# Furyton/Recommender-Baseline-Model

Hardware: AMD Instinct MI355X
Metric: training sequences/sec, SASRec L=200 d=128 at 1/2/4/8 MI355X; HR@10 parity (higher is better)
Workload: dtype bf16; 1 GPU; SASRec ML-1M shape (|items|=3416, seq_len=200, d=128, 2 blocks, 1 head, dropout 0.2); model=SASRec, global_batch=128, per_gpu_batch=128, seq_len=200, hidden=128, blocks=2, heads=1, num_items=3416, parallelism=dp1, hip_graph=True, bench_config=cfg2, sampler=host, steps_per_graph=10, full=False

## Files before the change

### include/recsys_hip.h

```cpp
#ifndef RECSYS_HIP_H
#define RECSYS_HIP_H
#include <stdint.h>
#ifdef __cplusplus
extern "C" {
#endif

#define RS_ERR_ARG 1001
#define RS_ERR_UNSUPPORTED 1002

typedef struct rs_epilogue {
  const float* bias;
  float alpha;
  int act;
  const void* aux;
  void* aux_out;
  int64_t ldaux;
  float drop_p;
  uint64_t drop_seed;
  const uint64_t* seed_base;
  int64_t drop_ld;
  const void* resid;
  int64_t ldres;
  const int64_t* rowmask_ids;
  int accumulate;
// ... 205 lines not shown
                        float* part, void* stream);
int rs_sas_block_boundary_fused(int64_t M, int64_t d);
int rs_sas_block_out_in(int64_t M, int64_t d, const void* o, const void* Q, const void* Wo, const float* bo, void* x1,
                        const float* ln_w, const float* ln_b, float eps, void* z, float* mean, float* rstd,
                        const void* W1, const float* b1, void* h1, const void* W2, const float* b2, void* xn,
                        const int64_t* ids, float drop_p, uint64_t salt1, uint64_t salt2, const uint64_t* seed_base,
                        const float* ln1_w, const float* ln1_b, float eps1, void* Qn, float* mean1, float* rstd1,
                        const void* Wq, const float* bq, void* q, const void* Wkv, const float* bkv, void* kv,
                        void* stream);
int rs_sas_block_in_out_bwd(int64_t M, int64_t d, const void* dq, const void* dkv, const void* dx1, const void* x,
                            const float* mean1, const float* rstd1, const float* ln1_w, const void* WinT, void* dx,
                            float* part1, const int64_t* ids, const void* h1, const void* x1, const float* mean2,
                            const float* rstd2, const float* ln2_w, const void* W2T, const void* W1T, const void* WoT,
                            void* dy2, void* da1, void* dx1o, void* dout, float* part2, float drop_p, uint64_t salt1,
                            uint64_t salt2, const uint64_t* seed_base, const void* o, float* delta, void* stream);
int rs_transpose_bf16(int64_t nmat, const int64_t* desc, int64_t max_tiles, const void* src, void* dst,
                      void* stream);

typedef struct {
  const void* dY; int64_t lddy;
  const void* X;  int64_t ldx;
  int64_t N, K;
  float* dW;
  float* db;
} rs_wgrad_problem;
typedef struct {
  const float* src; int64_t stride; int64_t splits; int64_t n; float* out;
} rs_reduce_segment;
int64_t rs_wgrad_grouped_slab_numel(int nprob, const rs_wgrad_problem* probs, int64_t M, int64_t rows_per_split);
int rs_wgrad_grouped_tile(int nprob, const rs_wgrad_problem* probs);
// ... 83 lines not shown
```

### recommender-baseline-model_amd/_lib.py

```python
import ctypes as C
import os

import torch

PKG = os.path.dirname(os.path.abspath(__file__))
LIB_PATH = os.path.join(PKG, "librecsys_hip.so" if not os.environ.get("RS_LIB_VARIANT")
                        else f"librecsys_hip.{os.environ['RS_LIB_VARIANT']}.so")

F32, BF16 = 0, 1

i32, i64, u64, f32, f64, vp = C.c_int, C.c_int64, C.c_uint64, C.c_float, C.c_double, C.c_void_p


class Epilogue(C.Structure):
    _fields_ = [
        ("bias", vp), ("alpha", f32), ("act", i32),
        ("aux", vp), ("aux_out", vp), ("ldaux", i64),
        ("drop_p", f32), ("drop_seed", u64), ("seed_base", vp), ("drop_ld", i64),
        ("resid", vp), ("ldres", i64),
        ("rowmask_ids", vp), ("accumulate", i32),
        ("post_drop_p", f32), ("post_drop_seed", u64), ("rows_dev", vp),
    ]


# ... 72 lines not shown
                              u64, u64, vp, vp, vp, vp, vp, vp, vp, i64, vp, vp, vp, vp, vp, vp, vp, vp, vp, vp],
    "rs_sas_block_in_embed": [i64, i64, vp, i64, vp, vp, f32, f32, u64, vp, vp, vp, vp, vp, vp, f32, vp, vp, vp, vp,
                              vp, vp, vp, vp, vp, vp],
    "rs_sas_block_out": [i64, i64, vp, vp, vp, vp, vp, vp, vp, f32, vp, vp, vp, vp, vp, vp, vp, vp, vp, vp, f32,
                         u64, u64, vp, vp],
    "rs_sas_block_out_bwd": [i64, i64, vp, vp, vp, vp, vp, vp, vp, vp, vp, vp, vp, vp, vp, vp, vp, f32, u64, u64,
                             vp, vp],
    "rs_sas_block_out_bwd_delta": [i64, i64, vp, vp, vp, vp, vp, vp, vp, vp, vp, vp, vp, vp, vp, vp, vp, f32, u64,
                                   u64, vp, vp, vp, vp],
    "rs_sas_block_in_bwd": [i64, i64, vp, vp, vp, vp, vp, vp, vp, vp, vp, vp, vp],
    "rs_sas_block_boundary_fused": [i64, i64],
    "rs_sas_block_out_in": [i64, i64, vp, vp, vp, vp, vp, vp, vp, f32, vp, vp, vp, vp, vp, vp, vp, vp, vp, vp, f32,
                            u64, u64, vp, vp, vp, f32, vp, vp, vp, vp, vp, vp, vp, vp, vp, vp],
    "rs_sas_block_in_out_bwd": [i64, i64, vp, vp, vp, vp, vp, vp, vp, vp, vp, vp, vp, vp, vp, vp, vp, vp, vp, vp, vp,
                                vp, vp, vp, vp, vp, f32, u64, u64, vp, vp, vp, vp],
    "rs_wgrad_grouped": [i32, C.POINTER(WgradProblem), i64, i64, vp, i64, i32, C.POINTER(ReduceSegment), vp],
    "rs_reduce_segments": [i32, C.POINTER(ReduceSegment), i32, vp],
    "rs_wgrad_grouped_slab_numel": [i32, C.POINTER(WgradProblem), i64, i64],
    "rs_wgrad_grouped_tile": [i32, C.POINTER(WgradProblem)],
    "rs_wgrad_grouped_tile_max": [i32, C.POINTER(WgradProblem), i32],
    "rs_wgrad_grouped_max": [i32, C.POINTER(WgradProblem), i64, i64, vp, i64, i32, C.POINTER(ReduceSegment), i32, vp],
    "rs_item_index_ws_bytes": [i32, i64, i64, i64],
    "rs_item_index_build": [i32, vp, vp, vp, i64, i64, i64, vp, i64, vp],
    "rs_item_index_layout": [i32, i64, i64, i64, C.POINTER(i64)],
    "rs_sas_head_fwd": [i64, i64, vp, vp, vp, f32, vp, vp, vp, vp, vp, vp, vp, vp, vp, vp],
    "rs_sas_head_finish": [i64, vp, vp, vp, vp],
    "rs_sas_head_bwd": [i64, i64, vp, vp, vp, vp, vp, vp, vp, vp, vp, vp, vp, vp, vp, vp, vp, vp, vp, vp, vp],
    "rs_item_grad": [vp, i32, i64, i64, i64, vp, f32, f32, u64, vp, vp, vp, vp, vp, vp],
    "rs_item_grad_marked": [vp, i32, i64, i64, i64, vp, f32, f32, u64, vp, vp, vp, vp, vp, vp, vp, vp],
    "rs_item_grad_f32": [vp, i32, i64, i64, i64, vp, f32, f32, u64, vp, vp, vp, vp, vp, vp],
# ... 65 lines not shown
```

### recommender-baseline-model_amd/csrc/rowchain.hip

```cpp
#include "common.h"
#include "../../include/recsys_hip.h"

namespace rc {

#ifdef RC_PROF
__device__ unsigned long long g_rc_prof[4096 * 8 * 16];
#define RCPROF(slot)                                                                                 \
  do {                                                                                               \
    if ((threadIdx.x & 63) == 0) g_rc_prof[(blockIdx.x * 8 + (threadIdx.x >> 6)) * 16 + (slot)] = wall_clock64(); \
  } while (0)
#else
#define RCPROF(slot) \
  do {               \
  } while (0)
#endif

#ifndef RC_HEAD_PREFETCH
#define RC_HEAD_PREFETCH 1
#endif

#ifndef RC_NOSTORE
#define RC_NOSTORE 0
#endif

// ... 114 lines not shown
  for (int j = 0; j < Lay<D>::J; ++j)
#pragma unroll
    for (int e = 0; e < 4; ++e) {
      const float u = x.v[j][e] - mu;
      q += u * u;
    }
  rs = 1.0f / sqrtf(row_sum(q) / (float)D + eps);
#pragma unroll
  for (int j = 0; j < Lay<D>::J; ++j) {
    const f32x4 w = vec4<D>(gw, j, g), b = vec4<D>(gb, j, g);
#pragma unroll
    for (int e = 0; e < 4; ++e) x.v[j][e] = (x.v[j][e] - mu) * rs * w[e] + b[e];
  }
}

__device__ __forceinline__ float row16_sum(float v) { return row16_sum_up(v); }

template <int D>
__device__ __forceinline__ void ln_bwd(Act<D>& dy, const Raw<D>& xr, bool valid, const float* gw, float mu, float a,
                                       float* red, int lane, int wave) {
  const int g = lane >> 4, cl = lane & 15;
  float* rw = red + wave * 2 * D;
  float sg = 0.f, sgu = 0.f;
#pragma unroll
  for (int j = 0; j < Lay<D>::J; ++j) {
    const f32x4 w = vec4<D>(gw, j, g);
#pragma unroll
    for (int e = 0; e < 4; ++e) {
      const float gy = valid ? dy.v[j][e] : 0.f;
      const float u = (float)xr.v[j >> 1][4 * (j & 1) + e] - mu;
      const float gq = gy * w[e];
      const float pg = row16_sum(gy * (u * a)), pb = row16_sum(gy);
      if (cl == 0) {
        rw[feat(j, g, e)] += pg;
        rw[D + feat(j, g, e)] += pb;
      }
      sg += gq;
      sgu += gq * u;
      dy.v[j][e] = gq;
    }
  }
  sg = row_sum(sg);
  sgu = row_sum(sgu);
  const float mg = sg / (float)D, coef = a * a * a * sgu / (float)D;
#pragma unroll
  for (int j = 0; j < Lay<D>::J; ++j) asm volatile("" : "+v"(dy.v[j]));
#pragma unroll
  for (int j = 0; j < Lay<D>::J; ++j)
#pragma unroll
    for (int e = 0; e < 4; ++e)
      dy.v[j][e] = a * (dy.v[j][e] - mg) - coef * ((float)xr.v[j >> 1][4 * (j & 1) + e] - mu);
}

__device__ __forceinline__ void ln_zero(float* red, int D, int lane, int wave) {
  for (int i = lane; i < 2 * D; i += 64) red[wave * 2 * D + i] = 0.f;
}
template <int D>
__device__ __forceinline__ void ln_partials(const float* red, float* part, int tid) {
  __syncthreads();
  if (tid < 2 * D) {
    const int which = tid / D, c = tid % D;
    float s = 0.f;
#pragma unroll
    for (int w = 0; w < NW; ++w) s += red[(w * 2 + which) * D + c];
    part[((int64_t)blockIdx.x * 2 + which) * D + c] = s;
  }
// ... 75 lines not shown
}

struct OutFwd {
  bf16 *x1, *z, *h1, *xn;
  float *mean, *rstd;
  const int64_t* ids;
  float drop_p, eps;
  uint32_t s1, s2;
};
__device__ __forceinline__ void drop4(float p, uint32_t s32, int64_t m, int D, int j, int g, float (&dm)[4]) {
  const uint64_t idx = (uint64_t)(m * D + feat(j, g, 0));
  drop_mul2(p, s32, idx, dm[0], dm[1]);
  drop_mul2(p, s32, idx + 2, dm[2], dm[3]);
}
template <int D>
__device__ __forceinline__ void fwd_out_a(const Raw<D>& orr, const Raw<D>& Qr, const Tile& T, const bf16* wo,
                                          const bf16* w1, const float* lv, const OutFwd& o, Raw<D>& zr, Raw<D>& hr,
                                          int lane) {
  const int g = lane >> 4;
  Act<D> acc;
  Raw<D> r;
  zero<D>(acc);
  mm<D>(wo, orr, acc, lane);
#pragma unroll
  for (int j = 0; j < Lay<D>::J; ++j) {
    const f32x4 bb = vec4<D>(lv, j, g);
#pragma unroll
    for (int e = 0; e < 4; ++e) acc.v[j][e] = acc.v[j][e] + bb[e] + (float)Qr.v[j >> 1][4 * (j & 1) + e];
  }
  round_act<D>(acc, r);
  if (!RC_NOSTORE) store_raw<D>(o.x1, D, T.m, T.ok, r, g);
  float mu, rs;
  ln_fwd<D>(acc, lv + D, lv + 2 * D, o.eps, g, mu, rs);
  round_act<D>(acc, zr);
  if (!RC_NOSTORE) store_raw<D>(o.z, D, T.m, T.ok, zr, g);
  if (T.ok && g == 0) {
    o.mean[T.m] = mu;
    o.rstd[T.m] = rs;
  }
  zero<D>(acc);
  mm<D>(w1, zr, acc, lane);
  const bool drop = o.drop_p > 0.f;
#pragma unroll
  for (int j = 0; j < Lay<D>::J; ++j) {
    float dm[4] = {1.f, 1.f, 1.f, 1.f};
    if (drop) drop4(o.drop_p, o.s1, T.m, D, j, g, dm);
    const f32x4 bb = vec4<D>(lv + 3 * D, j, g);
#pragma unroll
    for (int e = 0; e < 4; ++e) acc.v[j][e] = fmaxf(acc.v[j][e] + bb[e], 0.f) * dm[e];
  }
  round_act<D>(acc, hr);
  if (!RC_NOSTORE) store_raw<D>(o.h1, D, T.m, T.ok, hr, g);
}
template <int D>
__device__ __forceinline__ void fwd_out_b(const Raw<D>& hr, const Raw<D>& zr, const Tile& T, const bf16* w2,
                                          const float* lv, const OutFwd& o, Raw<D>& xr, int lane, bool keep) {
  const int g = lane >> 4;
  Act<D> acc;
  zero<D>(acc);
  mm<D>(w2, hr, acc, lane);
  const bool drop = o.drop_p > 0.f;
#pragma unroll
  for (int j = 0; j < Lay<D>::J; ++j) {
    float dm[4] = {1.f, 1.f, 1.f, 1.f};
    if (drop) drop4(o.drop_p, o.s2, T.m, D, j, g, dm);
    const f32x4 bb = vec4<D>(lv + 4 * D, j, g);
#pragma unroll
// ... 228 lines not shown
__device__ __forceinline__ float h_sigmoid(float z) { return 1.f / (1.f + __expf(-z)); }

template <int D>
__device__ __forceinline__ int64_t head_rows(const HeadArgs& h, const Tile& T, Raw<D>& er, Raw<D>& nr, int g) {
  const int64_t ip = h.pos[T.mc], in = h.neg[T.mc];
  load_raw<D>(er, h.E, D, ip, g);
  load_raw<D>(nr, h.E, D, in, g);
  return ip;
}
template <int D>
__device__ __forceinline__ void head_rows_at(const HeadArgs& h, int64_t ip, int64_t in, Raw<D>& er, Raw<D>& nr,
                                             int g) {
  load_raw<D>(er, h.E, D, ip, g);
  load_raw<D>(nr, h.E, D, in, g);
}
template <int D>
__device__ __forceinline__ void head_tile(const Raw<D>& xr, const Raw<D>& er, const Raw<D>& nr, int64_t ip,
                                          const Tile& T, const float* gl, const float* bl, const HeadArgs& h,
                                          float scale, float* red, float (&acc)[3], int lane, int wave) {
  const int g = lane >> 4;
  Act<D> y;
  to_act<D>(y, xr);
  float mu, rs;
  ln_fwd<D>(y, gl, bl, h.eps, g, mu, rs);
  Raw<D> fr;
  round_act<D>(y, fr);
  store_raw<D>(h.f, D, T.m, T.ok, fr, g);
  float dp = 0.f, dn = 0.f;
#pragma unroll
  for (int j = 0; j < Lay<D>::J; ++j)
#pragma unroll
    for (int e = 0; e < 4; ++e) {
      dp += y.v[j][e] * (float)er.v[j >> 1][4 * (j & 1) + e];
      dn += y.v[j][e] * (float)nr.v[j >> 1][4 * (j & 1) + e];
    }
  dp = row_sum(dp);
  dn = row_sum(dn);
  const bool valid = T.ok && ip != 0;
  const float gp = valid ? (h_sigmoid(dp) - 1.f) * scale : 0.f;
// ... 3 lines not shown
    h.nl[T.m] = dn;
    h.dpl[T.m] = gp;
    h.dnl[T.m] = gn;
    if (ip != 0) {
      acc[0] += h_softplus(-dp);
      acc[1] += h_softplus(dn);
      acc[2] += 1.f;
    }
  }
  Act<D> df;
#pragma unroll
  for (int j = 0; j < Lay<D>::J; ++j)
#pragma unroll
    for (int e = 0; e < 4; ++e)
      df.v[j][e] = gp * (float)er.v[j >> 1][4 * (j & 1) + e] + gn * (float)nr.v[j >> 1][4 * (j & 1) + e];
  ln_bwd<D>(df, xr, T.ok, gl, mu, rs, red, lane, wave);
  Raw<D> dr;
  round_act<D>(df, dr);
  store_raw<D>(h.dx, D, T.m, T.ok, dr, g);
}
__device__ __forceinline__ OutFwd out_fwd_of(const OutArgs& a) {
  const bool drop = a.drop_p > 0.f;
  return OutFwd{a.x1, a.z, a.h1, a.xn, a.mean, a.rstd, a.ids, a.drop_p, a.eps,
                drop ? seed32(eff_seed(a.salt1, a.seed_base)) : 0u, drop ? seed32(eff_seed(a.salt2, a.seed_base)) : 0u};
}

template <int D, bool HEAD>
__global__ __launch_bounds__(NT) void block_out_kernel(OutArgs a) {
  extern __shared__ __attribute__((aligned(16))) char smem[];
  typedef Smem<D, 3, 7, 1> L;
  constexpr int WB = Lay<D>::WBYTES;
  const float* lv = reinterpret_cast<const float*>(smem + L::W);
  float* red = reinterpret_cast<float*>(smem + L::V);
  constexpr bool head = HEAD;
// ... 327 lines not shown
  }
  asm volatile("" ::: "memory");
  if (has) {
    as_loaded<D>(dxr);
    bwd_out_a<D>(dxr, hr, T, wimg(w3), ob, dzr, dar, lane, T.ok && id != 0);
  }
  if constexpr (R::ON) __syncthreads();
  asm volatile("" ::: "memory");
  if (has)
    bwd_out_b<D>(dar, x1r, dzr, orr, T, mu2, rs2, wimg(R::ON ? w0 : w4), wimg(R::ON ? w1 : w5), lv + D, ob, red2,
                 lane, wave);
  ln_partials<D>(red, a.part, tid);
  ln_partials<D>(red2, b.part, tid);
}

static int g_ncu = 0;
static int64_t grid_for(int64_t M) {
  if (g_ncu == 0) {
    int dev = 0, n = 0;
    if (hipGetDevice(&dev) == hipSuccess && hipDeviceGetAttribute(&n, hipDeviceAttributeMultiprocessorCount, dev) ==
                                                 hipSuccess && n > 0)
      g_ncu = n;
    else
      g_ncu = 256;
  }
  const int64_t nt = (M + TR - 1) / TR;
  return nt < g_ncu ? nt : g_ncu;
}
template <int D> static size_t lds_fwd() { return Smem<D, 3, 5, 0>::BYTES; }
template <int D, bool HEAD> static size_t lds_out() {
// ... 19 lines not shown
  else if (d == 128) head ? launch_out_t<128, true>(a, s) : launch_out_t<128, false>(a, s);
  else return RS_ERR_UNSUPPORTED;
  return (int)hipGetLastError();
}

static bool boundary_fused(int64_t M, int64_t d) {
  return M > 0 && (d == 64 || d == 128) && (M + TR - 1) / TR <= grid_for(M) * NW;
}
template <int D>
static void launch_out_in_t(const OutArgs& a, const InArgs& b, hipStream_t s) {
  hipLaunchKernelGGL(block_out_in_kernel<D>, dim3((unsigned)grid_for(a.M)), dim3(NT), 0, s, a, b);
}
template <int D>
static void launch_in_out_bwd_t(const InBwdArgs& a, const OutBwdArgs& b, hipStream_t s) {
  hipLaunchKernelGGL(block_in_out_bwd_kernel<D>, dim3((unsigned)grid_for(a.M)), dim3(NT), 0, s, a, b);
}

__global__ __launch_bounds__(256) void transpose_bf16_kernel(const int64_t* __restrict__ desc, const __bf16* src,
                                                             __bf16* dst) {
  __shared__ __bf16 t[64][66];
  const int64_t* dsc = desc + 6 * blockIdx.y;
  const int64_t rows = dsc[0], cols = dsc[1];
  const int64_t tc = cdiv(cols, 64);
  const int64_t tr = blockIdx.x / tc, tcc = blockIdx.x % tc;
  if (tr * 64 >= rows) return;
  const __bf16* sp = src + dsc[2];
  __bf16* dp = dst + dsc[4];
  const int64_t lds = dsc[3], ldd = dsc[5];
  for (int e = threadIdx.x; e < 64 * 64; e += 256) {
    const int r = e / 64, c = e % 64;
// ... 189 lines not shown
    if (rc1) return rc1;
    return rs_sas_block_out_bwd_delta(M, d, dx, ids, h1, x1p, mean2, rstd2, ln2_w, W2T, W1T, WoT, dy2, da1, dx1p, dout,
                                      part2, drop_p, salt1, salt2, seed_base, o, delta, stream);
  }
  rc::InBwdArgs a = {M, (const __bf16*)dq, (const __bf16*)dkv, (const __bf16*)dx1, (const __bf16*)x, mean1, rstd1,
                     ln1_w, (const __bf16*)WinT, 3 * d, nullptr, part1};
  rc::OutBwdArgs b = {M, nullptr, ids, (const __bf16*)h1, (const __bf16*)x1p, mean2, rstd2, ln2_w,
                      (const __bf16*)W2T, (const __bf16*)W1T, (const __bf16*)WoT, (__bf16*)dy2, (__bf16*)da1,
                      (__bf16*)dx1p, (__bf16*)dout, part2, drop_p, salt1, salt2, seed_base, (const __bf16*)o, delta};
  hipStream_t s = (hipStream_t)stream;
  if (d == 64) rc::launch_in_out_bwd_t<64>(a, b, s);
  else rc::launch_in_out_bwd_t<128>(a, b, s);
  return (int)hipGetLastError();
}

int rs_transpose_bf16(int64_t nmat, const int64_t* desc, int64_t max_tiles, const void* src, void* dst,
                      void* stream) {
  if (nmat <= 0 || max_tiles <= 0) return RS_ERR_ARG;
  hipLaunchKernelGGL(rc::transpose_bf16_kernel, dim3((unsigned)max_tiles, (unsigned)nmat), dim3(256), 0,
                     (hipStream_t)stream, desc, (const __bf16*)src, (__bf16*)dst);
  return (int)hipGetLastError();
}

}
```

### recommender-baseline-model_amd/models/sas_model/sas.py

```python
import math
import os

import torch
import torch.nn as nn

from ... import ops
from ...engine_util import Workspace, as_ids, capture_event, compute_dtype, require_cuda, site_salt
from ...flat import FlatParams

LN_EPS = 1e-8
SAS_LOSSES = ("bce", "ce")


class PointWiseFeedForward(nn.Module):

    def __init__(self, hidden_units, dropout_rate):
        super().__init__()
        self.conv1 = nn.Conv1d(hidden_units, hidden_units, kernel_size=1)
        self.conv2 = nn.Conv1d(hidden_units, hidden_units, kernel_size=1)
        self.dropout_rate = dropout_rate


class SAS(nn.Module):
    def __init__(self, args):
# ... 133 lines not shown
        self.d = model.hidden
        self.L = model.num_blocks
        self.H = model.heads
        self.Dh = self.d // self.H
        self.p = float(model.dropout_rate)
        self.dt = model.cdtype
        self.dev = flat.device
        if self.dt == torch.bfloat16:
            flat.enable_bf16()
        self.ws = Workspace(self.dev)
        self.seed_base = torch.zeros(1, dtype=torch.int64, device=self.dev)
        self.external_seed = False
        self.adam_transposes = False
        self._wT = None
        self.boundary_fuse = os.environ.get("RS_SAS_BOUNDARY_FUSE", "1") != "0"
        salt0 = int(torch.randint(0, 2 ** 62, (1,)).item())
        self.salt = {"emb": site_salt(salt0, 0)}
        for i in range(self.L):
            self.salt[f"attn{i}"] = site_salt(salt0, 1 + 4 * i)
            self.salt[f"ffn1_{i}"] = site_salt(salt0, 2 + 4 * i)
            self.salt[f"ffn2_{i}"] = site_salt(salt0, 3 + 4 * i)

    def sync_compute_weights(self):
        f = self.flat
        if f.bf16 is not None:
            if not f.stale:
                ops.cast_bf16(f.data, f.bf16)
            else:
                a = 0
                for lo, hi in sorted(f.stale) + [(f.numel, f.numel)]:
# ... 148 lines not shown
            ops.sas_block_in(x, ln_w, ln_b, LN_EPS, Q, mu1, r1, Wq, bq, q, Wkv, bkv, kv)
        if after_first is not None:
            after_first()
        xs = [x]
        for i in range(L):
            b = lay[i]
            ops.attn_fwd(B, T, H, Dh, b["q"], b["kv"][:, :d], b["kv"][:, d:], b["o"], b["lse"], 1.0 / math.sqrt(Dh),
                         0, ids, p, self.salt[f"attn{i}"], sb)
            if i + 1 < L:
                ln_w, ln_b, Q, mu1, r1, Wq, bq, q, Wkv, bkv, kv = in_args(i + 1)
                if self.boundary_fuse:
                    ops.sas_block_out_in(out_args(i), ln_w, ln_b, LN_EPS, Q, mu1, r1, Wq, bq, q, Wkv, bkv, kv)
                else:
                    ops.sas_block_out(*out_args(i))
                    ops.sas_block_in(b["xn"], ln_w, ln_b, LN_EPS, Q, mu1, r1, Wq, bq, q, Wkv, bkv, kv)
            elif head is not None:
                ops.sas_block_out_head(out_args(i), *head)
            else:
                ops.sas_block_out(*out_args(i))
            xs.append(b["xn"])
        for i in range(L):
            b = lay[i]
            for k_ in ("Q", "mu1", "r1", "q", "kv", "o", "lse", "x1", "z", "mu2", "r2", "h1"):
                s[k_].append(b[k_])
            s["x"].append(xs[i])
        return xs[L]

    @property
    def fused_head(self):
        return ops.sas_block_fused_ok(self.d, self.dt)
# ... 5 lines not shown
        e = self._buf
        G = lambda n: self.flat.view(n, grad)
        slab = self.ws.get("slab", (ops.wgrad_slab_numel(M, 2 * d, d),), torch.float32)
        wln = self.ws.get("ln", (2 * 512 * d,), torch.float32)
        wat = self.ws.get("attn", (B * H * T,), torch.float32)

        fused = ops.sas_block_fused_ok(d, self.dt)
        if fused:
            ev, iws = s["side"] if "side" in s else self._side_prologue(ids, s["pos"], s["neg"])
        if fused:
            dx = e("dx", (M, d))
            lnh = self.ws.get("lnh", (2 * d * (-(-M // 64)),), torch.float32)
            E, gl = self.W("item_emb.weight"), self.Wf("last_layernorm.weight")
            stats = ()
            nb = -(-M // 64)
            if dpl is None and "head_in_block" in s:
                assert s["hdiv"] is divisor, "backward's divisor must be the one forward's head used"
                dx, dpl, dnl, lnh = s["hdx"], s["dpl"], s["dnl"], s["lnh"]
                nb = s["headp"].numel() // 3
                if loss_out is not None:
                    stats = (s["headp"], divisor, loss_out) + ((aux_out,) if aux_out is not None else ())
            elif dpl is None:
                dpl, dnl = e("dpl", (B, T), torch.float32), e("dnl", (B, T), torch.float32)
                ops.sas_head_bwd(s["headp"], divisor, loss_out, s["pl"], s["nl"], None, None, dpl, dnl, s["pos"],
                                 s["neg"], E, s["xL"], gl, s["muf"], s["rf"], dx, lnh)
            else:
                ops.sas_head_bwd(None, None, None, None, None, dpl, dnl, None, None, s["pos"], s["neg"], E, s["xL"],
                                 gl, s["muf"], s["rf"], dx, lnh)
            segs = ops.ln_partial_segments(lnh, M, d, G("last_layernorm.weight"), G("last_layernorm.bias"), nb=nb)
            if self._side_refreshed:
# ... 219 lines not shown
        if self._wT is None:
            self._wT = torch.empty(L * 6 * d * d, dtype=torch.bfloat16, device=self.dev)
            desc = []
            for i in range(L):
                base = i * 6 * d * d
                pre, fw = f"attention_layers.{i}.", f"forward_layers.{i}."
                for name, rows, off in ((pre + "in_proj_weight", 3 * d, 0), (pre + "out_proj.weight", d, 3 * d * d),
                                        (fw + "conv1.weight", d, 4 * d * d), (fw + "conv2.weight", d, 5 * d * d)):
                    desc.append([rows, d, self.flat.offsets[name], d, base + off, rows])
            self._wT_desc = torch.tensor(desc, dtype=torch.int64, device=self.dev)
            self._wT_desc_host = desc
            self._wT_tiles = max(-(-r // 64) * -(-c // 64) for r, c, *_ in desc)
        ops.transpose_bf16(self._wT_desc, self._wT_tiles, self.flat.bf16, self._wT)
        return self._wT

    def _backward_blocks_fused(self, s, dx, grad, extra_segs=(), tail=None, pos=None):
        B, T, p, ids, sb = s["B"], s["T"], s["p"], s["ids"], s["sb"]
        M, d, H, Dh, L = B * T, self.d, self.H, self.Dh, self.L
        e = self._buf
        G = lambda n: self.flat.view(n, grad)
        wT = self._wT.view(L, 6, d, d)
        nb = ops.sas_block_parts(M)
        lnp = self.ws.get("lnp", (L, 2, 2 * d * nb), torch.float32)
        wat = self.ws.get("attn", (B * H * T,), torch.float32)
        probs, segs = [], list(extra_segs)
        g = [dict(dy2=e("dy2", (M, d)), da1=e("da1", (M, d)), dx1=e("dx1", (M, d)), do=e("do", (M, d)),
                  dq=e("dq", (M, d)), dkv=e("dkv", (M, 2 * d))) for _ in range(L)]

        dl = [self.ws.get(f"attn_delta{i}", (B * H * T,), torch.float32) for i in range(L)] if H == 1 else None

        def out_bwd_args(i):
            return (ids, s["h1"][i], s["x1"][i], s["mu2"][i], s["r2"][i], self.Wf(f"forward_layernorms.{i}.weight"),
                    wT[i, 5], wT[i, 4], wT[i, 3], g[i]["dy2"], g[i]["da1"], g[i]["dx1"], g[i]["do"], lnp[i, 0], p,
                    self.salt[f"ffn1_{i}"], self.salt[f"ffn2_{i}"], sb, s["o"][i] if dl else None, dl[i] if dl else None)

        def in_bwd_args(i):
            return (g[i]["dq"], g[i]["dkv"], g[i]["dx1"], s["x"][i], s["mu1"][i], s["r1"][i],
                    self.Wf(f"attention_layernorms.{i}.weight"), wT[i, 0:3].reshape(d, 3 * d))

        ops.sas_block_out_bwd(dx, *out_bwd_args(L - 1))
        for i in reversed(range(L)):
            pre, fw = f"attention_layers.{i}.", f"forward_layers.{i}."
            dq, dkv, kv = g[i]["dq"], g[i]["dkv"], s["kv"][i]
            ops.attn_bwd(B, T, H, Dh, s["q"][i], kv[:, :d], kv[:, d:], s["o"][i], g[i]["do"], s["lse"][i], dq,
                         dkv[:, :d], dkv[:, d:], 1.0 / math.sqrt(Dh), 0, ids, p, self.salt[f"attn{i}"], sb,
                         dl[i] if dl else wat, delta_in=bool(dl))
            if i > 0 and self.boundary_fuse:
                dxi = None if ops.sas_block_boundary_fused(M, d) else e("dxi", (M, d))
                ops.sas_block_in_out_bwd(in_bwd_args(i), dxi, lnp[i, 1], out_bwd_args(i - 1))
            else:
                dxi = e("dxi", (M, d))
                ops.sas_block_in_bwd(*in_bwd_args(i), dxi, lnp[i, 1])
                if i > 0:
                    ops.sas_block_out_bwd(dxi, *out_bwd_args(i - 1))
            dx = dxi
# ... 52 lines not shown
```

### recommender-baseline-model_amd/ops.py

```python
import ctypes as C
import os

import torch

from . import _lib
from ._lib import BF16, F32, Epilogue, call, ptr, stream

ACT_NONE, ACT_RELU, ACT_GELU, ACT_RELU_BWD, ACT_GELU_BWD = (
    _lib.ACT_NONE, _lib.ACT_RELU, _lib.ACT_GELU, _lib.ACT_RELU_BWD, _lib.ACT_GELU_BWD)


STAMP_KINDS = {1: "attn_bwd", 2: "wgrad_grouped", 3: "vocab_ce_fwd"}


def kernel_stamps(buf, step, kinds=()):
    mask = sum(1 << k for k, n in STAMP_KINDS.items() if n in kinds)
    call("rs_kernel_stamps", ptr(buf), ptr(step), mask)


def read_kernel_stamps(buf, khz):
    import numpy as np
    h = buf.cpu().numpy().view(np.uint64)
    steps, marks, W = int(h[1]), int(h[2]), int(h[3])
    rec = h[4:4 + steps * marks * (1 + W)].reshape(steps, marks, 1 + W)
# ... 504 lines not shown
         ptr(seed_base), ptr(ln1_w), ptr(ln1_b), eps1, ptr(Qn), ptr(mean1), ptr(rstd1), ptr(Wq), ptr(bq), ptr(q),
         ptr(Wkv), ptr(bkv), ptr(kv), stream())


def sas_block_in_out_bwd(in_args, dx, part1, out_args):
    dq, dkv, dx1, x, mean1, rstd1, ln1_w, WinT = in_args
    (ids, h1, x1, mean2, rstd2, ln2_w, W2T, W1T, WoT, dy2, da1, dx1o, dout, part2, drop_p, salt1, salt2,
     seed_base, o, delta) = out_args
    M, d = dq.shape
    call("rs_sas_block_in_out_bwd", M, d, ptr(dq), ptr(dkv), ptr(dx1), ptr(x), ptr(mean1), ptr(rstd1), ptr(ln1_w),
         ptr(WinT), ptr(dx), ptr(part1), ptr(ids), ptr(h1), ptr(x1), ptr(mean2), ptr(rstd2), ptr(ln2_w), ptr(W2T),
         ptr(W1T), ptr(WoT), ptr(dy2), ptr(da1), ptr(dx1o), ptr(dout), ptr(part2), drop_p, salt1, salt2,
         ptr(seed_base), ptr(o), ptr(delta), stream())


def touched_rows_ws_numel(rows):
    return int(_lib.lib().rs_touched_rows_ws_numel(rows))


def touched_rows(ids, rows, flags, index, count, ws):
    call("rs_touched_rows", ptr(ids), ids.numel(), rows, ptr(flags), ptr(index), ptr(count), ptr(ws), stream())


def rows_pack(src, index, count, compact):
    rows, d = src.shape
    call("rs_rows_pack", ptr(src), rows, d, ptr(index), ptr(count), ptr(compact), compact.shape[0], stream())


def rows_unpack(dst, index, compact):
    rows, d = dst.shape
# ... 250 lines not shown
```

Measured before the change: 481,300 sequences/s.

## Fuse last block output, BCE head, and first backward step into one kernel

New measurement: 498,200 sequences/s, median of 6. +3.5%, better.

```diff
diff --git a/include/recsys_hip.h b/include/recsys_hip.h
--- a/include/recsys_hip.h
+++ b/include/recsys_hip.h
@@ -243,6 +243,15 @@
                             const float* rstd2, const float* ln2_w, const void* W2T, const void* W1T, const void* WoT,
                             void* dy2, void* da1, void* dx1o, void* dout, float* part2, float drop_p, uint64_t salt1,
                             uint64_t salt2, const uint64_t* seed_base, const void* o, float* delta, void* stream);
+int rs_sas_block_out_head_bwd(int64_t M, int64_t d, const void* o, const void* Q, const void* Wo, const float* bo,
+                              void* x1, const float* ln_w, const float* ln_b, float eps, void* z, float* mean,
+                              float* rstd, const void* W1, const float* b1, void* h1, const void* W2, const float* b2,
+                              void* xn, const int64_t* ids, float drop_p, uint64_t salt1, uint64_t salt2,
+                              const uint64_t* seed_base, const void* E, const int64_t* pos, const int64_t* neg,
+                              const float* lnl_w, const float* lnl_b, const int* count_parts, int64_t ncount,
+                              const float* divisor, void* f, float* pl, float* nl, float* dpl, float* dnl, void* dx,
+                              float* lnpart, float* part, const void* W2T, const void* W1T, const void* WoT, void* dy2,
+                              void* da1, void* dx1, void* dout, float* part2, float* delta, void* stream);
 int rs_transpose_bf16(int64_t nmat, const int64_t* desc, int64_t max_tiles, const void* src, void* dst,
                       void* stream);
 
diff --git a/recommender-baseline-model_amd/_lib.py b/recommender-baseline-model_amd/_lib.py
--- a/recommender-baseline-model_amd/_lib.py
+++ b/recommender-baseline-model_amd/_lib.py
@@ -110,6 +110,9 @@
                             u64, u64, vp, vp, vp, f32, vp, vp, vp, vp, vp, vp, vp, vp, vp, vp],
     "rs_sas_block_in_out_bwd": [i64, i64, vp, vp, vp, vp, vp, vp, vp, vp, vp, vp, vp, vp, vp, vp, vp, vp, vp, vp, vp,
                                 vp, vp, vp, vp, vp, f32, u64, u64, vp, vp, vp, vp],
+    "rs_sas_block_out_head_bwd": [i64, i64, vp, vp, vp, vp, vp, vp, vp, f32, vp, vp, vp, vp, vp, vp, vp, vp, vp, vp,
+                                  f32, u64, u64, vp, vp, vp, vp, vp, vp, vp, i64, vp, vp, vp, vp, vp, vp, vp, vp, vp,
+                                  vp, vp, vp, vp, vp, vp, vp, vp, vp, vp],
     "rs_wgrad_grouped": [i32, C.POINTER(WgradProblem), i64, i64, vp, i64, i32, C.POINTER(ReduceSegment), vp],
     "rs_reduce_segments": [i32, C.POINTER(ReduceSegment), i32, vp],
     "rs_wgrad_grouped_slab_numel": [i32, C.POINTER(WgradProblem), i64, i64],
diff --git a/recommender-baseline-model_amd/csrc/rowchain.hip b/recommender-baseline-model_amd/csrc/rowchain.hip
--- a/recommender-baseline-model_amd/csrc/rowchain.hip
+++ b/recommender-baseline-model_amd/csrc/rowchain.hip
@@ -152,9 +152,47 @@
   }
 }
 
+template <int D>
+__device__ __forceinline__ void ln_fwd_head(Act<D>& x, const float* gw, const float* gb, float eps, int g, float& mu,
+                                            float& rs) {
+  float s = 0.f;
+#pragma unroll
+  for (int j = 0; j < Lay<D>::J; ++j)
+#pragma unroll
+    for (int e = 0; e < 4; ++e) s += x.v[j][e];
+  mu = row_sum(s) / (float)D;
+  float q = 0.f, u0 = 0.f;
+#pragma unroll
+  for (int j = 0; j < Lay<D>::J; ++j)
+#pragma unroll
+    for (int e = 0; e < 4; ++e) {
+      const float u = x.v[j][e] - mu;
+      if (j == 0 && e == 0) {
+        u0 = u;
+      } else if (j == 0 && e == 1) {
+        float sq = u * u;
+        asm volatile("" : "+v"(sq));
+        q = __builtin_fmaf(u0, u0, sq);
+      } else if ((j & 1) == 0 && e < 2) {
+        q = __builtin_fmaf(u, u, q);
+      } else {
+        float sq = u * u;
+        asm volatile("" : "+v"(sq));
+        q += sq;
+      }
+    }
+  rs = 1.0f / sqrtf(row_sum(q) / (float)D + eps);
+#pragma unroll
+  for (int j = 0; j < Lay<D>::J; ++j) {
+    const f32x4 w = vec4<D>(gw, j, g), b = vec4<D>(gb, j, g);
+#pragma unroll
+    for (int e = 0; e < 4; ++e) x.v[j][e] = (x.v[j][e] - mu) * rs * w[e] + b[e];
+  }
+}
+
 __device__ __forceinline__ float row16_sum(float v) { return row16_sum_up(v); }
 
-template <int D>
+template <int D, bool HEAD_FORM = false>
 __device__ __forceinline__ void ln_bwd(Act<D>& dy, const Raw<D>& xr, bool valid, const float* gw, float mu, float a,
                                        float* red, int lane, int wave) {
   const int g = lane >> 4, cl = lane & 15;
@@ -173,8 +211,13 @@
         rw[feat(j, g, e)] += pg;
         rw[D + feat(j, g, e)] += pb;
       }
-      sg += gq;
-      sgu += gq * u;
+      if constexpr (HEAD_FORM) {
+        sg = __builtin_fmaf(gy, w[e], sg);
+        sgu = __builtin_fmaf(u, gq, sgu);
+      } else {
+        sg += gq;
+        sgu += gq * u;
+      }
       dy.v[j][e] = gq;
     }
   }
@@ -186,8 +229,21 @@
 #pragma unroll
   for (int j = 0; j < Lay<D>::J; ++j)
 #pragma unroll
-    for (int e = 0; e < 4; ++e)
-      dy.v[j][e] = a * (dy.v[j][e] - mg) - coef * ((float)xr.v[j >> 1][4 * (j & 1) + e] - mu);
+    for (int e = 0; e < 4; ++e) {
+      const float u = (float)xr.v[j >> 1][4 * (j & 1) + e] - mu;
+      if constexpr (HEAD_FORM) {
+        float p1 = a * (dy.v[j][e] - mg), p2 = coef * u;
+        if ((j & 1) == 0 && e < 2) {
+          asm volatile("" : "+v"(p1), "+v"(p2));
+          dy.v[j][e] = p1 - p2;
+        } else {
+          asm volatile("" : "+v"(p2));
+          dy.v[j][e] = __builtin_fmaf(a, dy.v[j][e] - mg, -p2);
+        }
+      } else {
+        dy.v[j][e] = a * (dy.v[j][e] - mg) - coef * u;
+      }
+    }
 }
 
 __device__ __forceinline__ void ln_zero(float* red, int D, int lane, int wave) {
@@ -293,12 +349,11 @@
   drop_mul2(p, s32, idx + 2, dm[2], dm[3]);
 }
 template <int D>
-__device__ __forceinline__ void fwd_out_a(const Raw<D>& orr, const Raw<D>& Qr, const Tile& T, const bf16* wo,
-                                          const bf16* w1, const float* lv, const OutFwd& o, Raw<D>& zr, Raw<D>& hr,
-                                          int lane) {
+__device__ __forceinline__ void fwd_out_a_x(const Raw<D>& orr, const Raw<D>& Qr, const Tile& T, const bf16* wo,
+                                            const bf16* w1, const float* lv, const OutFwd& o, Raw<D>& zr, Raw<D>& hr,
+                                            int lane, Raw<D>& r, float& mu, float& rs) {
   const int g = lane >> 4;
   Act<D> acc;
-  Raw<D> r;
   zero<D>(acc);
   mm<D>(wo, orr, acc, lane);
 #pragma unroll
@@ -309,7 +364,6 @@
   }
   round_act<D>(acc, r);
   if (!RC_NOSTORE) store_raw<D>(o.x1, D, T.m, T.ok, r, g);
-  float mu, rs;
   ln_fwd<D>(acc, lv + D, lv + 2 * D, o.eps, g, mu, rs);
   round_act<D>(acc, zr);
   if (!RC_NOSTORE) store_raw<D>(o.z, D, T.m, T.ok, zr, g);
@@ -330,6 +384,14 @@
   }
   round_act<D>(acc, hr);
   if (!RC_NOSTORE) store_raw<D>(o.h1, D, T.m, T.ok, hr, g);
+}
+template <int D>
+__device__ __forceinline__ void fwd_out_a(const Raw<D>& orr, const Raw<D>& Qr, const Tile& T, const bf16* wo,
+                                          const bf16* w1, const float* lv, const OutFwd& o, Raw<D>& zr, Raw<D>& hr,
+                                          int lane) {
+  Raw<D> r;
+  float mu, rs;
+  fwd_out_a_x<D>(orr, Qr, T, wo, w1, lv, o, zr, hr, lane, r, mu, rs);
 }
 template <int D>
 __device__ __forceinline__ void fwd_out_b(const Raw<D>& hr, const Raw<D>& zr, const Tile& T, const bf16* w2,
@@ -588,15 +650,17 @@
   load_raw<D>(er, h.E, D, ip, g);
   load_raw<D>(nr, h.E, D, in, g);
 }
-template <int D>
-__device__ __forceinline__ void head_tile(const Raw<D>& xr, const Raw<D>& er, const Raw<D>& nr, int64_t ip,
-                                          const Tile& T, const float* gl, const float* bl, const HeadArgs& h,
-                                          float scale, float* red, float (&acc)[3], int lane, int wave) {
+template <int D, bool STORE_DX>
+__device__ __forceinline__ void head_tile_x(const Raw<D>& xr, const Raw<D>& er, const Raw<D>& nr, int64_t ip,
+                                            const Tile& T, const float* gl, const float* bl, const HeadArgs& h,
+                                            float scale, float* red, float (&acc)[3], int lane, int wave,
+                                            Raw<D>& dxr) {
   const int g = lane >> 4;
   Act<D> y;
   to_act<D>(y, xr);
   float mu, rs;
-  ln_fwd<D>(y, gl, bl, h.eps, g, mu, rs);
+  if constexpr (STORE_DX) ln_fwd<D>(y, gl, bl, h.eps, g, mu, rs);
+  else ln_fwd_head<D>(y, gl, bl, h.eps, g, mu, rs);
   Raw<D> fr;
   round_act<D>(y, fr);
   store_raw<D>(h.f, D, T.m, T.ok, fr, g);
@@ -630,10 +694,18 @@
 #pragma unroll
     for (int e = 0; e < 4; ++e)
       df.v[j][e] = gp * (float)er.v[j >> 1][4 * (j & 1) + e] + gn * (float)nr.v[j >> 1][4 * (j & 1) + e];
-  ln_bwd<D>(df, xr, T.ok, gl, mu, rs, red, lane, wave);
+  ln_bwd<D, !STORE_DX>(df, xr, T.ok, gl, mu, rs, red, lane, wave);
   Raw<D> dr;
   round_act<D>(df, dr);
-  store_raw<D>(h.dx, D, T.m, T.ok, dr, g);
+  if (STORE_DX) store_raw<D>(h.dx, D, T.m, T.ok, dr, g);
+  dxr = dr;
+}
+template <int D>
+__device__ __forceinline__ void head_tile(const Raw<D>& xr, const Raw<D>& er, const Raw<D>& nr, int64_t ip,
+                                          const Tile& T, const float* gl, const float* bl, const HeadArgs& h,
+                                          float scale, float* red, float (&acc)[3], int lane, int wave) {
+  Raw<D> dr;
+  head_tile_x<D, true>(xr, er, nr, ip, T, gl, bl, h, scale, red, acc, lane, wave, dr);
 }
 __device__ __forceinline__ OutFwd out_fwd_of(const OutArgs& a) {
   const bool drop = a.drop_p > 0.f;
@@ -991,6 +1063,123 @@
   ln_partials<D>(red2, b.part, tid);
 }
 
+struct TurnArgs {
+  OutArgs a;
+  OutBwdArgs b;
+};
+typedef const __attribute__((address_space(4))) TurnArgs* TurnArgsPtr;
+__device__ __forceinline__ TurnArgsPtr turn_args_late() {
+  TurnArgsPtr kp = (TurnArgsPtr)__builtin_amdgcn_kernarg_segment_ptr();
+  asm volatile("" : "+s"(kp));
+  return kp;
+}
+template <int D>
+__global__ __launch_bounds__(NT) void block_out_head_bwd_kernel(TurnArgs k) {
+  const OutArgs& a = k.a;
+  typedef Roll<D> R;
+  RC_BOUNDARY_SLOTS(D);
+  __shared__ __attribute__((aligned(16))) float lv[7 * D];
+  __shared__ __attribute__((aligned(16))) float red[NW * 2 * D], red2[NW * 2 * D];
+  __shared__ float hred[4][NW];
+  const int tid = threadIdx.x, lane = tid & 63, wave = __builtin_amdgcn_readfirstlane(tid >> 6), g = lane >> 4,
+            cl = lane & 15;
+  RCPROF(0);
+  const TileRange tr = tiles_of_wave(n_tiles(a.M), wave);
+  const bool has = tr.first < tr.end;
+  const Tile T = tile_of(has ? tr.first : 0, a.M, cl);
+  const OutFwd of = out_fwd_of(a);
+  Raw<D> orr, Qr;
+  int64_t id = 0, ip = 0, in = 0;
+  if (has) {
+    load_raw<D>(orr, a.o, D, T.mc, g);
+    load_raw<D>(Qr, a.Q, D, T.mc, g);
+    id = a.ids[T.mc];
+    ip = a.h.pos[T.mc];
+    in = a.h.neg[T.mc];
+  }
+  stage_slot<D>(w0, a.Wo, D, wave, lane);
+  stage_slot<D>(w1, a.W1, D, wave, lane);
+  stage_slot<D>(w2, a.W2, D, wave, lane);
+  stage_slot<D>(w3, k.b.W2T, D, wave, lane);
+  if constexpr (!R::ON) {
+    stage_slot<D>(w4, k.b.W1T, D, wave, lane);
+    stage_slot<D>(w5, k.b.WoT, D, wave, lane);
+  }
+  {
+    const float* const V[7] = {a.bo, a.ln_w, a.ln_b, a.b1, a.b2, a.h.gl, a.h.bl};
+    stage_v<D, 7>(lv, V, tid);
+  }
+  ln_zero(red, D, lane, wave);
+  ln_zero(red2, D, lane, wave);
+  float hacc[3] = {0.f, 0.f, 0.f};
+  {
+    int c = 0;
+    for (int i = tid; i < a.h.ncnt; i += NT) c += a.h.cnt_parts[i];
+    c = (int)wave_sum((float)c);
+    if (lane == 0) hred[3][wave] = (float)c;
+  }
+  __syncthreads();
+  float hscale;
+  {
+    float c = 0.f;
+#pragma unroll
+    for (int w = 0; w < NW; ++w) c += hred[3][w];
+    hscale = 1.f / (a.h.divisor ? *a.h.divisor : c);
+  }
+  asm volatile("" : "+v"(id), "+v"(ip), "+v"(in));
+  RCPROF(1);
+  Raw<D> zr, hr, x1r, xr, er, nr, dr, dzr, dar;
+  float mu2 = 0.f, rs2 = 0.f;
+  if (has) {
+    fwd_out_a_x<D>(orr, Qr, T, wimg(w0), wimg(w1), lv, of, zr, hr, lane, x1r, mu2, rs2);
+    head_rows_at<D>(a.h, ip, in, er, nr, g);
+  }
+  RCPROF(2);
+  if constexpr (R::ON) {
+    __syncthreads();
+    const TurnArgsPtr kp = turn_args_late();
+    stage_slot<D>(w0, kp->b.W1T, D, wave, lane);
+    stage_slot<D>(w1, kp->b.WoT, D, wave, lane);
+  }
+  asm volatile("" ::: "memory");
+  const TurnArgsPtr kb = turn_args_late();
+  const OutBwd ob = {kb->b.dy2, kb->b.da1, kb->b.dx1, kb->b.dout, kb->b.delta, a.ids, a.drop_p, of.s1, of.s2};
+  if (has) {
+    const bool keep = T.ok && id != 0;
+    fwd_out_b<D>(hr, zr, T, wimg(w2), lv, of, xr, lane, keep);
+    RCPROF(4);
+    head_tile_x<D, false>(xr, er, nr, ip, T, lv + 5 * D, lv + 6 * D, a.h, hscale, red, hacc, lane, wave, dr);
+    RCPROF(6);
+    asm volatile("" ::: "memory");
+    as_loaded<D>(dr);
+    as_loaded<D>(hr);
+    bwd_out_a<D>(dr, hr, T, wimg(w3), ob, dzr, dar, lane, keep);
+  }
+  if constexpr (R::ON) __syncthreads();
+  asm volatile("" ::: "memory");
+  if (has) {
+    as_loaded<D>(x1r);
+    as_loaded<D>(orr);
+    asm volatile("" : "+v"(mu2), "+v"(rs2));
+    bwd_out_b<D>(dar, x1r, dzr, orr, T, mu2, rs2, wimg(R::ON ? w0 : w4), wimg(R::ON ? w1 : w5), lv + D, ob, red2, lane,
+                 wave);
+  }
+  RCPROF(5);
+#pragma unroll
+  for (int k = 0; k < 3; ++k) {
+    const float v = wave_sum(hacc[k]);
+    if (lane == 0) hred[k][wave] = v;
+  }
+  ln_partials<D>(red, a.h.lnpart, tid);
+  ln_partials<D>(red2, kb->b.part, tid);
+  if (tid < 3) {
+    float v = 0.f;
+#pragma unroll
+    for (int w = 0; w < NW; ++w) v += hred[tid][w];
+    a.h.part[blockIdx.x * 3 + tid] = v;
+  }
+}
+
 static int g_ncu = 0;
 static int64_t grid_for(int64_t M) {
   if (g_ncu == 0) {
@@ -1040,6 +1229,10 @@
 template <int D>
 static void launch_in_out_bwd_t(const InBwdArgs& a, const OutBwdArgs& b, hipStream_t s) {
   hipLaunchKernelGGL(block_in_out_bwd_kernel<D>, dim3((unsigned)grid_for(a.M)), dim3(NT), 0, s, a, b);
+}
+template <int D>
+static void launch_out_head_bwd_t(const OutArgs& a, const OutBwdArgs& b, hipStream_t s) {
+  hipLaunchKernelGGL(block_out_head_bwd_kernel<D>, dim3((unsigned)grid_for(a.M)), dim3(NT), 0, s, TurnArgs{a, b});
 }
 
 __global__ __launch_bounds__(256) void transpose_bf16_kernel(const int64_t* __restrict__ desc, const __bf16* src,
@@ -1259,6 +1452,40 @@
   return (int)hipGetLastError();
 }
 
+int rs_sas_block_out_head_bwd(int64_t M, int64_t d, const void* o, const void* Q, const void* Wo, const float* bo,
+                              void* x1, const float* ln_w, const float* ln_b, float eps, void* z, float* mean,
+                              float* rstd, const void* W1, const float* b1, void* h1, const void* W2, const float* b2,
+                              void* xn, const int64_t* ids, float drop_p, uint64_t salt1, uint64_t salt2,
+                              const uint64_t* seed_base, const void* E, const int64_t* pos, const int64_t* neg,
+                              const float* lnl_w, const float* lnl_b, const int* count_parts, int64_t ncount,
+                              const float* divisor, void* f, float* pl, float* nl, float* dpl, float* dnl, void* dx,
+                              float* lnpart, float* part, const void* W2T, const void* W1T, const void* WoT, void* dy2,
+                              void* da1, void* dx1, void* dout, float* part2, float* delta, void* stream) {
+  if (M <= 0 || !E || !pos || !neg || !count_parts || ncount <= 0 || !f || !lnpart || !part) return RS_ERR_ARG;
+  if (d != 64 && d != 128) return RS_ERR_UNSUPPORTED;
+  if (!rc::boundary_fused(M, d)) {
+    if (!dx) return RS_ERR_ARG;
+    const int rc1 = rs_sas_block_out_head(M, d, o, Q, Wo, bo, x1, ln_w, ln_b, eps, z, mean, rstd, W1, b1, h1, W2, b2, xn,
+                                          ids, drop_p, salt1, salt2, seed_base, E, pos, neg, lnl_w, lnl_b, count_parts,
+                                          ncount, divisor, f, pl, nl, dpl, dnl, dx, lnpart, part, stream);
+    if (rc1) return rc1;
+    return rs_sas_block_out_bwd_delta(M, d, dx, ids, h1, x1, mean, rstd, ln_w, W2T, W1T, WoT, dy2, da1, dx1, dout,
+                                      part2, drop_p, salt1, salt2, seed_base, delta ? o : nullptr, delta, stream);
+  }
+  rc::OutArgs a = {M, (const __bf16*)o, (const __bf16*)Q, (const __bf16*)Wo, bo, (__bf16*)x1, ln_w, ln_b, eps,
+                   (__bf16*)z, mean, rstd, (const __bf16*)W1, b1, (__bf16*)h1, (const __bf16*)W2, b2, (__bf16*)xn,
+                   ids, drop_p, salt1, salt2, seed_base,
+                   rc::HeadArgs{(const __bf16*)E, pos, neg, lnl_w, lnl_b, eps, count_parts, (int)ncount, divisor,
+                                (__bf16*)f, pl, nl, dpl, dnl, nullptr, lnpart, part}};
+  rc::OutBwdArgs b = {M, nullptr, ids, (const __bf16*)h1, (const __bf16*)x1, mean, rstd, ln_w, (const __bf16*)W2T,
+                      (const __bf16*)W1T, (const __bf16*)WoT, (__bf16*)dy2, (__bf16*)da1, (__bf16*)dx1, (__bf16*)dout,
+                      part2, drop_p, salt1, salt2, seed_base, (const __bf16*)o, delta};
+  hipStream_t s = (hipStream_t)stream;
+  if (d == 64) rc::launch_out_head_bwd_t<64>(a, b, s);
+  else rc::launch_out_head_bwd_t<128>(a, b, s);
+  return (int)hipGetLastError();
+}
+
 int rs_transpose_bf16(int64_t nmat, const int64_t* desc, int64_t max_tiles, const void* src, void* dst,
                       void* stream) {
   if (nmat <= 0 || max_tiles <= 0) return RS_ERR_ARG;
diff --git a/recommender-baseline-model_amd/models/sas_model/sas.py b/recommender-baseline-model_amd/models/sas_model/sas.py
--- a/recommender-baseline-model_amd/models/sas_model/sas.py
+++ b/recommender-baseline-model_amd/models/sas_model/sas.py
@@ -171,6 +171,7 @@
         self.adam_transposes = False
         self._wT = None
         self.boundary_fuse = os.environ.get("RS_SAS_BOUNDARY_FUSE", "1") != "0"
+        self.turnaround_fuse = os.environ.get("RS_SAS_TURNAROUND_FUSE", "1") != "0"
         salt0 = int(torch.randint(0, 2 ** 62, (1,)).item())
         self.salt = {"emb": site_salt(salt0, 0)}
         for i in range(self.L):
@@ -349,6 +350,12 @@
                 else:
                     ops.sas_block_out(*out_args(i))
                     ops.sas_block_in(b["xn"], ln_w, ln_b, LN_EPS, Q, mu1, r1, Wq, bq, q, Wkv, bkv, kv)
+            elif head is not None and self.turnaround_fuse:
+                if self._side_refreshed:
+                    torch.cuda.current_stream().wait_event(s["side"][0])
+                tb = self._out_bwd_bufs(s, i)
+                ops.sas_block_out_head_bwd(out_args(i), head, *tb["args"])
+                s["turnaround"] = tb
             elif head is not None:
                 ops.sas_block_out_head(out_args(i), *head)
             else:
@@ -384,6 +391,7 @@
             E, gl = self.W("item_emb.weight"), self.Wf("last_layernorm.weight")
             stats = ()
             nb = -(-M // 64)
+            assert dpl is None or "turnaround" not in s, "the forward already ran the backward of its own BCE gradient"
             if dpl is None and "head_in_block" in s:
                 assert s["hdiv"] is divisor, "backward's divisor must be the one forward's head used"
                 dx, dpl, dnl, lnh = s["hdx"], s["dpl"], s["dnl"], s["lnh"]
@@ -633,6 +641,16 @@
         ops.transpose_bf16(self._wT_desc, self._wT_tiles, self.flat.bf16, self._wT)
         return self._wT
 
+    def _out_bwd_bufs(self, s, i):
+        B, T = s["B"], s["T"]
+        M, d, H, L = B * T, self.d, self.H, self.L
+        e = self._buf
+        wT = self._wT.view(L, 6, d, d)
+        lnp = self.ws.get("lnp", (L, 2, 2 * d * ops.sas_block_parts(M)), torch.float32)
+        g = dict(dy2=e("dy2", (M, d)), da1=e("da1", (M, d)), dx1=e("dx1", (M, d)), do=e("do", (M, d)))
+        dl = self.ws.get(f"attn_delta{i}", (B * H * T,), torch.float32) if H == 1 else None
+        return dict(g=g, args=(wT[i, 5], wT[i, 4], wT[i, 3], g["dy2"], g["da1"], g["dx1"], g["do"], lnp[i, 0], dl))
+
     def _backward_blocks_fused(self, s, dx, grad, extra_segs=(), tail=None, pos=None):
         B, T, p, ids, sb = s["B"], s["T"], s["p"], s["ids"], s["sb"]
         M, d, H, Dh, L = B * T, self.d, self.H, self.Dh, self.L
@@ -645,6 +663,9 @@
         probs, segs = [], list(extra_segs)
         g = [dict(dy2=e("dy2", (M, d)), da1=e("da1", (M, d)), dx1=e("dx1", (M, d)), do=e("do", (M, d)),
                   dq=e("dq", (M, d)), dkv=e("dkv", (M, 2 * d))) for _ in range(L)]
+        turn = s.get("turnaround")
+        if turn is not None:
+            g[L - 1].update(turn["g"])
 
         dl = [self.ws.get(f"attn_delta{i}", (B * H * T,), torch.float32) for i in range(L)] if H == 1 else None
 
@@ -657,7 +678,8 @@
             return (g[i]["dq"], g[i]["dkv"], g[i]["dx1"], s["x"][i], s["mu1"][i], s["r1"][i],
                     self.Wf(f"attention_layernorms.{i}.weight"), wT[i, 0:3].reshape(d, 3 * d))
 
-        ops.sas_block_out_bwd(dx, *out_bwd_args(L - 1))
+        if turn is None:
+            ops.sas_block_out_bwd(dx, *out_bwd_args(L - 1))
         for i in reversed(range(L)):
             pre, fw = f"attention_layers.{i}.", f"forward_layers.{i}."
             dq, dkv, kv = g[i]["dq"], g[i]["dkv"], s["kv"][i]
diff --git a/recommender-baseline-model_amd/ops.py b/recommender-baseline-model_amd/ops.py
--- a/recommender-baseline-model_amd/ops.py
+++ b/recommender-baseline-model_amd/ops.py
@@ -542,6 +542,22 @@
          ptr(seed_base), ptr(o), ptr(delta), stream())
 
 
+def sas_block_out_head_bwd(out_args, head_args, W2T, W1T, WoT, dy2, da1, dx1, dout, part2, delta=None):
+    (o, Q, Wo, bo, x1, ln_w, ln_b, eps, z, mean, rstd, W1, b1, h1, W2, b2, xn, ids, drop_p, salt1, salt2,
+     seed_base) = out_args
+    E, pos, neg, lnl_w, lnl_b, count_parts, divisor, f, pl, nl, dpl, dnl, dx, lnpart, part = head_args
+    M, d = o.shape
+    G = sas_block_grid(M)
+    assert part.numel() == 3 * G and lnpart.numel() >= 2 * d * G and count_parts.dtype == torch.int32
+    assert part2.numel() >= 2 * d * G
+    call("rs_sas_block_out_head_bwd", M, d, ptr(o), ptr(Q), ptr(Wo), ptr(bo), ptr(x1), ptr(ln_w), ptr(ln_b), eps,
+         ptr(z), ptr(mean), ptr(rstd), ptr(W1), ptr(b1), ptr(h1), ptr(W2), ptr(b2), ptr(xn), ptr(ids), drop_p, salt1,
+         salt2, ptr(seed_base), ptr(E), ptr(pos), ptr(neg), ptr(lnl_w), ptr(lnl_b), ptr(count_parts),
+         count_parts.numel(), ptr(divisor), ptr(f), ptr(pl), ptr(nl), ptr(dpl), ptr(dnl), ptr(dx), ptr(lnpart),
+         ptr(part), ptr(W2T), ptr(W1T), ptr(WoT), ptr(dy2), ptr(da1), ptr(dx1), ptr(dout), ptr(part2), ptr(delta),
+         stream())
+
+
 def touched_rows_ws_numel(rows):
     return int(_lib.lib().rs_touched_rows_ws_numel(rows))
 
```
